# Godotcoffee/AlignGraph2

Hardware: AMD Instinct MI355X
Metric: aligned-read-bases/sec through PAGraph build+traverse (higher is better)
Workload: dtype u32

## Files before the change

aligngraph2_amd/capi.py:

```python
import ctypes as C

import numpy as np

CONSTANTS = {
    "PAG_OK": 0, "PAG_EINVAL": -22, "PAG_ENOMEM": -12, "PAG_ENODEV": -19, "PAG_ERANGE": -34, "PAG_EFAULT": -14, "PAG_EDOM": -33,
    "PAG_NONE": 0xFFFFFFFF,
    "PAG_ALN_REV_STRAND": 1, "PAG_ALN_WALK_BACK": 2, "PAG_ALN_ELIGIBLE": 4,
    "PAG_ORIENT_NONE": -1, "PAG_ORIENT_REVERSE": 0, "PAG_ORIENT_FORWARD": 1, "PAG_ORIENT_BOTH": 2,
    "PAG_TRAVEL_RENDER_DUMPS": 1, "PAG_TRAVEL_RENDER_SEQS": 2,
}
globals().update(CONSTANTS)

DTYPES = {
    "pag_aln": np.dtype([("query", "<u4"), ("target", "<u4"), ("t_begin", "<u4"), ("t_end", "<u4"), ("q_start", "<u4"),
                         ("t_start", "<u4"), ("n_cols", "<u4"), ("n_valid", "<u4"), ("diff_off", "<u8"), ("flags", "<u4"),
                         ("reserved", "<u4")]),
    "pag_ctg": np.dtype([("len", "<u4"), ("selected", "<u4"), ("single_base", "<u4"), ("multi", "<u4"), ("map_off", "<u8")]),
    "pag_ref": np.dtype([("len", "<u4"), ("accepted", "<u4"), ("single_base", "<u4"), ("reserved", "<u4")]),
    "pag_raw_aln": np.dtype([("query", "<u4"), ("target", "<u4"), ("score", "<u8"), ("q_begin", "<u8"), ("q_end", "<u8"),
                             ("t_begin", "<u8"), ("t_end", "<u8"), ("diff_off", "<u8"), ("n_cols", "<u4"), ("n_emit", "<u4"),
                             ("n_radv", "<u4"), ("forward", "<u4")]),
    "pag_path_node": np.dtype([("code", "<u4"), ("ctg", "<u4"), ("ref", "<u4"), ("cnt", "<u2"), ("reserved", "<u2"),
                               ("step", "<i4"), ("vid", "<u4")]),
}

_u32, _i32, _u64, _f64, _vp = C.c_uint32, C.c_int32, C.c_uint64, C.c_double, C.c_void_p


class PagSeqs(C.Structure):
    _c_name_ = "pag_seqs"
    _fields_ = [("n_seqs", _u64), ("byte_off", _vp), ("len", _vp), ("packed", _vp), ("packed_bytes", _u64)]


class PagAlnDb(C.Structure):
    _c_name_ = "pag_aln_db"
    _fields_ = [("n_aln", _u64), ("aln", _vp), ("query_off", _vp), ("diff", _vp), ("n_diff_words", _u64)]


class PagBuildInput(C.Structure):
    _c_name_ = "pag_build_input"
    _fields_ = [("on_device", _u32), ("n_threads", _u32), ("reads", PagSeqs), ("emit_order", _vp), ("read_to_ctg", PagAlnDb),
                ("read_to_ref", PagAlnDb), ("n_ctgs", _u64), ("ctgs", _vp), ("ctg_ent_off", _vp), ("n_ctg_ent_off", _u64),
                ("ctg_ent", _vp), ("n_ctg_ent", _u64), ("n_refs", _u64), ("refs", _vp), ("eps", _u32), ("cov_filter", _u32),
                ("outer_sample", _u32), ("topk_ctg", _i32), ("topk_ref", _i32), ("reserved", _u32)]


class PagRawDb(C.Structure):
    _c_name_ = "pag_raw_db"
    _fields_ = [("n", _u64), ("rec", _vp), ("diff", _vp), ("n_diff_words", _u64)]


class PagRawInput(C.Structure):
    _c_name_ = "pag_raw_input"
    _fields_ = [("bulk_on_device", _u32), ("n_threads", _u32), ("reads", PagSeqs), ("read_to_ctg", PagRawDb),
                ("read_to_ref", PagRawDb), ("ctg_to_ref", PagRawDb), ("n_ctgs", _u64), ("ctg_len", _vp), ("ctg_selected", _vp),
                ("ctg_forward", _vp), ("n_refs", _u64), ("ref_len", _vp), ("ref_accepted", _vp), ("read_to_ctg_ratio", _f64),
                ("read_to_ref_ratio", _f64), ("eps", _u32), ("cov_filter", _u32), ("outer_sample", _u32), ("topk_ctg", _i32),
                ("topk_ref", _i32), ("reserved", _u32)]


class BuildStats(C.Structure):
    _c_name_ = "pag_build_stats"
    _fields_ = [("merge_edge", _u64 * 2), ("total_pos", _u64 * 2), ("merge_pos", _u64 * 2), ("n_tuples", _u64 * 2),
                ("n_edges", _u64 * 2), ("n_nodes", _u64), ("n_pos", _u64), ("n_uniq_edges", _u64), ("ms_extract", _f64),
                ("ms_sort", _f64), ("ms_cluster", _f64), ("ms_edges", _f64), ("ms_total", _f64), ("ms_sort_kernel", _f64),
                ("sort_records", _u64)]

    def counts(self):
        return (self.merge_edge[0], self.total_pos[0], self.merge_pos[0], self.merge_edge[1], self.total_pos[1],
                self.merge_pos[1])


class Csr(C.Structure):
    _c_name_ = "pag_csr"
    _fields_ = [("n_nodes", _u64), ("n_pos", _u64), ("n_edges", _u64), ("node_code", _vp), ("pos_off", _vp), ("pos_ctg", _vp),
                ("pos_ref", _vp), ("pos_cnt", _vp), ("edge_off", _vp), ("edge_to", _vp), ("edge_step", _vp)]


class ShardSlice(C.Structure):
    _c_name_ = "pag_shard_slice"
    _fields_ = [("n_t", _u64), ("n_e", _u64), ("tkey", _vp), ("tval", _vp), ("tseg", _vp), ("tcnt", _vp), ("ekey", _vp),
                ("eval", _vp), ("eseg", _vp), ("stats", BuildStats)]


class Region(C.Structure):
    _c_name_ = "pag_region"
    _fields_ = [("n_ctg_iv", _u64), ("ctg_iv", _vp), ("n_ref_iv", _u64), ("ref_iv", _vp), ("ref_open", _vp)]


class TravelParams(C.Structure):
    _c_name_ = "pag_travel_params"
    _fields_ = [("ref_threads", _u32), ("reserved", _u32), ("deviation", _u64), ("error_rate", _f64), ("start_split", _f64),
                ("min_len", _u64)]


class TravelStats(C.Structure):
    _c_name_ = "pag_travel_stats"
    _fields_ = [("ms_compact", _f64), ("ms_walk", _f64), ("ms_total", _f64), ("rounds", _u64), ("jobs", _u64),
                ("walk_steps", _u64), ("classify_calls", _u64), ("probes", _u64), ("records", _u64)]


class PagSucc(C.Structure):
    _c_name_ = "pag_succ"
    _fields_ = [("code", _u32), ("step", _u32), ("pos", _u64), ("grade", _u32), ("ctg_similar", _u32)]


class CnsAln(C.Structure):
    _c_name_ = "pag_cns_aln"
    _fields_ = [("str_off", _u64), ("len", _u32), ("start", _u32), ("weight", _i32), ("reserved", _u32)]


class CnsPart(C.Structure):
    _c_name_ = "pag_cns_part"
    _fields_ = [("bb_off", _u64), ("bb_len", _u32), ("n_aln", _u32), ("aln_first", _u64), ("node_cap", _u32),
                ("edge_cap", _u32), ("aux_cap", _u32), ("out_cap", _u32)]


class KmerCountResult(C.Structure):
    _c_name_ = "pag_kmer_count_result"
    _fields_ = [("min_abundance", _u64), ("n_solid", _u64), ("n_kmers_counted", _u64), ("ms_count", _f64), ("ms_select", _f64)]


class TraverseStats(C.Structure):
    _c_name_ = "pagh_traverse_stats"
    _fields_ = [("n_contigs", _u64), ("n_path_nodes", _u64), ("n_path_bases", _u64), ("n_chains_emitted", _u64),
                ("n_fasta_bases", _u64), ("path_checksum", _u64), ("ms_export", _f64), ("ms_traverse", _f64), ("ms_total", _f64),
                ("ms_successors", _f64), ("ms_walk", _f64), ("walk_rounds", _u64), ("walk_jobs", _u64), ("walk_steps", _u64),
                ("walk_classifications", _u64)]


STRUCTS = {s._c_name_: s for s in (PagSeqs, PagAlnDb, PagBuildInput, PagRawDb, PagRawInput, BuildStats, Csr, ShardSlice, Region,
                                   TravelParams, TravelStats, PagSucc, CnsAln, CnsPart, KmerCountResult, TraverseStats)}

NOT_MIRRORED = {}

_int, _i64, _cs = C.c_int, C.c_int64, C.c_char_p
_u64p, _i64p, _intp = C.POINTER(_u64), C.POINTER(_i64), C.POINTER(_int)
_stats, _slice, _region = C.POINTER(BuildStats), C.POINTER(ShardSlice), C.POINTER(Region)
_traverse = [_vp, _u32, _vp, _vp, _vp, _vp, _vp, _u32, _u64, _u64, _cs, _cs, _u32, _vp]
_cns = [_int, _cs, _u64, _vp, _u64, _vp, _u64, _cs, _cs, _u64, _i32, _vp, _u64, _vp, _vp, _vp]

SIGNATURES = {
    "pag_create": (_vp, [_vp, _u64, _u32, _int, _intp]),
    "pag_create_from_bitmap": (_vp, [_vp, _u64, _u32, _int, _int, _intp]),
    "pag_destroy": (None, [_vp]),
    "pag_solid_count": (_u64, [_vp]),
    "pag_reset": (_int, [_vp]),
    "pag_process": (_int, [_vp, _vp, _vp]),
    "pag_prepare": (_int, [_vp, _vp, _vp]),
    "pag_shard_extract": (_int, [_vp, _vp, _u32, _u32, _u64p]),
    "pag_shard_extract_range": (_int, [_vp, _vp, _u64, _u64, _u32, _u64p]),
    "pag_shard_take": (_int, [_vp, _vp, _vp, _vp, _vp]),
    "pag_shard_take_part": (_int, [_vp, _u64, _u64, _vp, _vp, _u64, _u64, _vp, _vp]),
    "pag_shard_build": (_int, [_vp, _vp, _vp, _u64, _u64, _vp, _vp, _u64, _u64, _u32, _stats]),
    "pag_shard_export": (_int, [_vp, _slice]),
    "pag_shard_take_slice": (_int, [_vp, _vp, _vp, _vp, _vp, _vp, _vp, _vp]),
    "pag_shard_import": (_int, [_vp, _slice, _u32, _stats]),
    "pag_shard_select": (_int, [_vp, _region, _slice]),
    "pag_shard_set_region": (_int, [_vp, _region]),
    "pag_shard_release_build": (_int, [_vp]),
    "pag_shard_adopt": (_int, [_vp, _u64, _u64, _stats]),
    "pag_comm_create": (_vp, [_int, _int, _cs, _int, _cs, _intp]),
    "pag_comm_destroy": (None, [_vp]),
    "pag_comm_rank": (_int, [_vp]),
    "pag_comm_world": (_int, [_vp]),
    "pag_comm_bytes_sent": (_u64, [_vp]),
    "pag_comm_abort": (None, [_vp, _cs]),
    "pag_comm_barrier": (_int, [_vp]),
    "pag_comm_all_gather": (_int, [_vp, _vp, _u64, _vp]),
    "pag_comm_gather_v": (_int, [_vp, _vp, _u64, _int, _vp, _u64, _vp, _vp]),
    "pag_comm_all_to_all_v": (_int, [_vp, _vp, _vp, _vp, _vp]),
    "pag_shard_run": (_int, [_vp, _vp, _vp, _vp, _stats]),
    "pag_csr_sizes": (_int, [_vp, _u64p, _u64p, _u64p]),
    "pag_export_csr": (_int, [_vp, _vp]),
    "pag_travel_prepare": (_int, [_vp, _vp, _vp, _u64, _vp, _vp]),
    "pag_travel_prepare_for": (_int, [_vp, _vp, _vp, _vp, _u64, _vp, _vp]),
    "pag_travel_view_sizes": (_int, [_vp, _vp, _vp, _vp, _vp, _vp, _vp]),
    "pag_travel": (_int, [_vp, _vp, _vp, _vp, _u64, _vp, _vp]),
    "pag_successors": (_i64, [_vp, _u32, _u64, _vp, _u64]),
    "pag_travel_path": (_vp, [_vp, _u64, _u64p]),
    "pag_travel_path_oriented": (_vp, [_vp, _u64, _int, _u64p]),
    "pag_reserve_walk_arena": (_int, [_vp, _u64]),
    "pag_render_dump_lines": (_int, [_vp, _u64, _u32, _vp, _u64, _vp, _u64, _vp, _u64, _u64p, _int]),
    "pag_travel_dump_text": (_vp, [_vp, _u64, _int, _u64p]),
    "pag_render_path_sequence": (_int, [_vp, _u64, _u32, _vp, _vp, _u64, _f64, _vp, _u64, _u64p, _int]),
    "pag_travel_seq_sources": (_int, [_vp, _vp]),
    "pag_travel_seq_text": (_vp, [_vp, _u64, _int, _u64p]),
    "pag_pack_text_seqs": (_int, [_vp, _int, _u64, _vp, _vp, _u64, _vp, _vp, _u64, _int]),
    "pag_classify_columns": (_int, [_vp, _int, _u64, _vp, _vp, _vp, _vp, _vp, _u64, _vp, _u64, _vp, _vp, _int]),
    "pag_classify_columns_host": (_int, [_vp, _u64, _vp, _vp, _vp, _vp, _vp, _u64, _vp, _u64, _vp, _vp, _int]),
    "pag_cns_consensus": (_int, _cns),
    "pag_cns_consensus_wave": (_int, _cns),
    "pag_kmer_count": (_int, [_vp, _int, _u32, _f64, _int, _vp, _int, _vp]),
    "pag_last_error": (_cs, []),
    "pag_device_available": (_int, []),
    "pag_device_warm": (_int, [_int]),
    "pagh_traverse": (_int, _traverse),
    "pagh_traverse_begin": (_int, [_vp, _u32, _vp, _vp, _vp, _vp, _vp, _u32, _u64, _u64, _cs, _cs, _u32]),
    "pagh_traverse_end": (_int, [_vp, _vp]),
    "pagh_assemble_paths": (_int, [_vp, _u32, _vp, _vp, _vp, _vp, _vp, _vp, _vp, _u32, _u64, _u64, _cs, _cs, _u32, _vp]),
    "pagh_assemble_paths_text": (_int, [_vp, _u32, _vp, _vp, _vp, _vp, _vp, _vp, _vp, _vp, _vp, _u32, _u64, _u64, _cs, _cs, _u32,
                                        _vp]),
    "pagh_assemble_paths_seq": (_int, [_vp, _u32, _vp, _vp, _vp, _vp, _vp, _vp, _vp, _vp, _vp, _vp, _vp, _u32, _u64, _u64, _cs, _cs,
                                       _u32, _vp]),
    "pagh_release": (None, [_vp]),
    "pagh_last_error": (_cs, []),
    "pag_debug_edit_distance": (_u64, [_cs, _cs]),
    "pag_debug_mapper_d2s": (_u64, [_vp, _u64, _i64, _i64]),
    "pag_debug_mapper_s2d": (None, [_vp, _u64, _u64, _i64p, _i64p]),
    "pag_debug_mapper_extra": (_u64, [_vp, _u64]),
    "pag_debug_succ_sizes": (_int, [_vp, _vp, _vp]),
    "pag_debug_succ": (_int, [_vp, _vp, _vp]),
    "pag_debug_trav_vertices": (_int, [_vp, _vp, _vp]),
    "pag_debug_stream_sizes": (_int, [_vp, _u64p, _u64p]),
    "pag_debug_streams": (_int, [_vp, _vp, _vp, _vp, _vp]),
    "pag_debug_cov_filter": (_int, [_vp, _u64, _vp, _u64, _u32, _vp, _int]),
    "pag_debug_predicates": (_int, [_vp, _u64, _f64, _vp, _vp, _int]),
    "pag_debug_predicates_tab": (_int, [_vp, _u64, _f64, _vp, _vp, _int, _vp]),
    "pagh_debug_classify_columns": (None, [_cs, _u64, _cs, _u64, _vp, _vp, _vp, _int]),
    "pagh_debug_pack_bases": (None, [_cs, _u64, _vp, _int]),
}


def bind(lib, rename=None):
    for name, (restype, argtypes) in SIGNATURES.items():
        sym = rename(name) if rename else name
        fn = getattr(lib, sym, None) if sym else None
        if fn is not None:
            fn.restype = restype
            fn.argtypes = list(argtypes)
    return lib
```

aligngraph2_amd/csrc/hip/k5_travel_host.hip:

```cpp
#include <algorithm>
#include <atomic>
#include <chrono>
#include <cmath>
#include <cstdio>
#include <cstdlib>
#include <cstring>
#include <deque>
#include <string>
#include <thread>
#include <unordered_set>
#include <vector>

#include "pag_graph_impl.hpp"
#include "pagraph_debug.h"
#include "walk_config.hpp"
#include "walk_stitch.hpp"
#include "walker_grid.hpp"

using namespace pagdev;

namespace {

#include "trav_prepare_host.hpp"
#include "walk_session_jobs.hpp"
#include "walk_session_rounds.hpp"
#include "walk_session_loop.hpp"


}


extern "C" {

uint64_t pag_debug_edit_distance(const char *a, const char *b) { return edit_distance(a, b); }
uint64_t pag_debug_mapper_d2s(const uint32_t *len, uint64_t n, int64_t idx, int64_t pos) { return Mapper(len, n).dualToSingle(idx, pos); }
void pag_debug_mapper_s2d(const uint32_t *len, uint64_t n, uint64_t single, int64_t *idx, int64_t *pos) {
    auto d = Mapper(len, n).singleToDual(single);
    *idx = d.first;
    *pos = d.second;
}
uint64_t pag_debug_mapper_extra(const uint32_t *len, uint64_t n) { return Mapper(len, n).starts.back(); }

const pag_path_node *pag_travel_path_oriented(const pag_graph *g, uint64_t ctg_index, int forward, uint64_t *len) {
    const uint64_t slot = 2 * ctg_index + (forward ? 0 : 1);
    if (!g || slot >= g->path_valid.size() || !g->path_valid[slot]) {
        if (len) *len = 0;
        return nullptr;
    }
    if (len) *len = g->path_len[slot];
    if (slot < g->path_ptr.size() && g->path_ptr[slot]) return g->path_ptr[slot];
    return g->path_store + g->path_off[slot];
}

const char *pag_travel_dump_text(const pag_graph *g, uint64_t ctg_index, int forward, uint64_t *bytes) {
    const uint64_t slot = 2 * ctg_index + (forward ? 0 : 1);
    if (bytes) *bytes = 0;
    if (!g || slot >= g->path_valid.size() || !g->path_valid[slot] || slot >= g->text_ptr.size() || !g->text_ptr[slot]) return nullptr;
    if (bytes) *bytes = g->text_len[slot];
    return g->text_ptr[slot];
}

const char *pag_travel_seq_text(const pag_graph *g, uint64_t ctg_index, int forward, uint64_t *bytes) {
    const uint64_t slot = 2 * ctg_index + (forward ? 0 : 1);
    if (bytes) *bytes = 0;
    if (!g || slot >= g->path_valid.size() || !g->path_valid[slot] || slot >= g->seq_ptr.size() || !g->seq_ptr[slot]) return nullptr;
    if (bytes) *bytes = g->seq_len[slot];
    return g->seq_ptr[slot];
}
int pag_travel_seq_sources(pag_graph *g, const pag_seqs *refs) {
    if (!g) return PAG_EINVAL;
    g->seq_refs = refs;
    return PAG_OK;
}

const pag_path_node *pag_travel_path(const pag_graph *g, uint64_t ctg_index, uint64_t *len) {
    if (g && 2 * ctg_index + 1 < g->path_valid.size() && !g->path_valid[2 * ctg_index]) return pag_travel_path_oriented(g, ctg_index, 0, len);
    return pag_travel_path_oriented(g, ctg_index, 1, len);
}

int pag_debug_succ_sizes(const pag_graph *g, uint64_t *n_pos, uint64_t *n_succ) {
    if (!g || !g->tg_ready || !n_pos || !n_succ) return PAG_EINVAL;
    *n_pos = g->tg.n_pos;
    *n_succ = g->tg.n_succ;
    return PAG_OK;
}
int pag_debug_succ(const pag_graph *g, uint32_t *succ_off, void *recs) {
    if (!g || !g->tg_ready || !succ_off || !recs) return PAG_EINVAL;
    PAG_HIP_TRY(hipSetDevice(g->device));
    PAG_HIP_TRY(hipMemcpy(succ_off, g->tg.succ_off, (g->tg.n_pos + 1) * 4, hipMemcpyDeviceToHost));
    PAG_HIP_TRY(hipMemcpy(recs, g->tg.succ, g->tg.n_succ * sizeof(SuccRec), hipMemcpyDeviceToHost));
    return PAG_OK;
}

int pag_debug_trav_vertices(const pag_graph *g, uint32_t *code, uint64_t *pos) {
    if (!g || !g->tg_ready || !code || !pos) return PAG_EINVAL;
    PAG_HIP_TRY(hipSetDevice(g->device));
    const TravGraph &G = g->tg;
    std::vector<uint32_t> uold(G.n_pos), vnode(G.n_pos), ncode(G.n_nodes);
    PAG_HIP_TRY(hipMemcpy(uold.data(), G.uold, G.n_pos * 4, hipMemcpyDeviceToHost));
    PAG_HIP_TRY(hipMemcpy(vnode.data(), G.vnode, G.n_pos * 4, hipMemcpyDeviceToHost));
    PAG_HIP_TRY(hipMemcpy(ncode.data(), G.ncode, G.n_nodes * 4, hipMemcpyDeviceToHost));
    PAG_HIP_TRY(hipMemcpy(pos, G.upos, G.n_pos * 8, hipMemcpyDeviceToHost));
    for (uint64_t u = 0; u < G.n_pos; ++u) code[u] = ncode[vnode[uold[u]]];
    return PAG_OK;
}

int64_t pag_successors(const pag_graph *g, uint32_t code, uint64_t pos, pag_succ *out, uint64_t cap) {
    if (!g || !g->tg_ready || (!out && cap)) return PAG_EINVAL;
    PAG_HIP_TRY(hipSetDevice(g->device));
    if (g->view_pruned || g->regional) {
        set_error("pag_successors: the prepared view was cut for given traversals (pag_travel_prepare_for / a regional graph): its lists are restricted to what those traversals can examine");
        return PAG_ERANGE;
    }
    void *d = nullptr;
    const uint64_t room = std::min<uint64_t>(cap, g->tg.n_succ);
    PAG_HIP_TRY(hipMalloc(&d, 16 + room * sizeof(pag_succ)));
    unsigned long long *d_n = (unsigned long long *)d;
    void *d_recs = (char *)d + 16;
    int rc = trav_successors_of(g->tg, code, pos, d_recs, room, d_n, g->stream);
    unsigned long long n = 0;
    if (rc == PAG_OK && (hipMemcpyAsync(&n, d_n, 8, hipMemcpyDeviceToHost, g->stream) != hipSuccess || hipStreamSynchronize(g->stream) != hipSuccess)) rc = PAG_EFAULT;
    if (rc == PAG_OK && n == ~0ull) {
        set_error("pag_successors: the graph holds no vertex with that k-mer and position");
        rc = PAG_EINVAL;
    } else if (rc == PAG_OK && n == ~1ull) {
        set_error("pag_successors: that vertex's list is a marker record");
        rc = PAG_ERANGE;
    } else if (rc == PAG_OK && std::min<uint64_t>(n, room) &&
               hipMemcpy(out, d_recs, std::min<uint64_t>(n, room) * sizeof(pag_succ), hipMemcpyDeviceToHost) != hipSuccess) {
        rc = PAG_EFAULT;
    }
    hipFree(d);
    return rc == PAG_OK ? (int64_t)n : rc;
}

int pag_travel_prepare(pag_graph *g, const pag_seqs *ctgs, const uint32_t *ref_len, uint64_t n_refs, const pag_travel_params *prm, double *ms) {
    return pag_travel_prepare_for(g, ctgs, nullptr, ref_len, n_refs, prm, ms);
}
int pag_travel_prepare_for(pag_graph *g, const pag_seqs *ctgs, const int32_t *orient, const uint32_t *ref_len, uint64_t n_refs,
                           const pag_travel_params *prm, double *ms) {
    if (!g || !ctgs || !prm || (!ref_len && n_refs)) return PAG_EINVAL;
    PAG_HIP_TRY(hipSetDevice(g->device));
    TravGraph G{};
    return trav_prepare_graph(g, ctgs->len, ctgs->n_seqs, ref_len, n_refs, prm->deviation, prm->error_rate, &G, ms, orient, prm->start_split);
}
int pag_travel_view_sizes(const pag_graph *g, uint64_t *n_nodes, uint64_t *n_pos, uint64_t *n_edges, uint64_t *n_succ, int *cut, uint64_t *fallbacks) {
    if (!g || !g->tg_ready) return PAG_EINVAL;
    if (n_nodes) *n_nodes = g->view_counts[0];
    if (n_pos) *n_pos = g->view_counts[1];
    if (n_edges) *n_edges = g->view_counts[2];
    if (n_succ) *n_succ = g->tg.n_succ;
    if (cut) *cut = g->view_pruned ? 1 : 0;
    if (fallbacks) *fallbacks = g->view_fallbacks;
    return PAG_OK;
}

static int travel_once(pag_graph *g, const pag_seqs *ctgs, const int32_t *orient, const uint32_t *ref_len, uint64_t n_refs,
                       const pag_travel_params *prm, pag_travel_stats *stats);
int pag_travel(pag_graph *g, const pag_seqs *ctgs, const int32_t *orient, const uint32_t *ref_len, uint64_t n_refs,
               const pag_travel_params *prm, pag_travel_stats *stats) {
    if (!g || !ctgs || !orient || !prm || (!ref_len && n_refs)) return PAG_EINVAL;
    int rc = travel_once(g, ctgs, orient, ref_len, n_refs, prm, stats);
    if (rc == PAG_ERANGE && g->view_pruned && !g->regional) {
        if (WalkConfig::from_env().timing) std::fprintf(stderr, "[timing] a walk left the view: %s; walking again on the whole graph\n", pag_last_error());
        g->view_off = true;
        g->tg_ready = false;
        g->view_fallbacks += 1;
        rc = travel_once(g, ctgs, orient, ref_len, n_refs, prm, stats);
    }
    g->seq_refs = nullptr;
    return rc;
}
static int travel_once(pag_graph *g, const pag_seqs *ctgs, const int32_t *orient, const uint32_t *ref_len, uint64_t n_refs,
                       const pag_travel_params *prm, pag_travel_stats *stats) {
    WalkSession W(g, ctgs, orient, ref_len, n_refs, prm, stats);
    return W.run();
}


}
```

aligngraph2_amd/csrc/hip/k5_view.hip:

```cpp
#include <algorithm>
#include <cmath>
#include <cstring>
#include <string>
#include <vector>

#include "pag_device.hpp"
#include "pag_travel.hpp"
#include "trav_device.hpp"

namespace pagdev {

__device__ __forceinline__ bool iv_contains(const uint32_t *__restrict__ iv, uint32_t n, uint32_t x, uint32_t *which = nullptr) {
    if (!n) return false;
    uint32_t lo = 0, hi = n;
    while (hi - lo > 1) {
        const uint32_t mid = (lo + hi) >> 1;
        if (iv[2 * mid] <= x) lo = mid;
        else hi = mid;
    }
    if (which) *which = lo;
    return x >= iv[2 * lo] && x < iv[2 * lo + 1];
}
constexpr uint32_t ZONE_LDS = 2048;
__global__ void k_zone_bands(const uint64_t *__restrict__ tval, uint64_t T, const uint32_t *__restrict__ zones, uint32_t n_z,
                             uint32_t *__restrict__ lo, uint32_t *__restrict__ hi) {
    __shared__ uint32_t s_lo[ZONE_LDS], s_hi[ZONE_LDS], s_z[2 * ZONE_LDS];
    const bool lds = n_z <= ZONE_LDS;
    if (lds) {
        for (uint32_t z = threadIdx.x; z < n_z; z += blockDim.x) {
            s_lo[z] = 0xFFFFFFFFu;
            s_hi[z] = 0u;
            s_z[2 * z] = zones[2 * z];
            s_z[2 * z + 1] = zones[2 * z + 1];
        }
        __syncthreads();
    }
    const uint32_t z_first = n_z ? zones[0] : 0u, z_last = n_z ? zones[2 * n_z - 1] : 0u;
    for (uint64_t i = (uint64_t)blockIdx.x * blockDim.x + threadIdx.x; i < T; i += (uint64_t)gridDim.x * blockDim.x) {
        const uint64_t p = tval[i];
        const uint32_t c = (uint32_t)(p >> 32), r = (uint32_t)p;
        uint32_t z;
        if (c < z_first || c >= z_last || r == 0u) continue;
        if (!(lds ? iv_contains(s_z, n_z, c, &z) : iv_contains(zones, n_z, c, &z))) continue;
        if (lds) {
            atomicMin(&s_lo[z], r);
            atomicMax(&s_hi[z], r);
        } else {
            atomicMin(&lo[z], r);
            atomicMax(&hi[z], r);
        }
    }
    if (lds) {
        __syncthreads();
        for (uint32_t z = threadIdx.x; z < n_z; z += blockDim.x)
            if (s_hi[z] != 0u) {
                atomicMin(&lo[z], s_lo[z]);
                atomicMax(&hi[z], s_hi[z]);
            }
    }
}
constexpr uint32_t PRUNE_LDS = 4096;
constexpr uint32_t VC_T = 256, VC_R = 8, VC_TILE = VC_T * VC_R, VC_W = VC_T / 64;
__global__ __launch_bounds__(VC_T) void k_view_mark(const uint32_t *__restrict__ tkey, const uint64_t *__restrict__ tval, const uint32_t *__restrict__ tseg,
                                                    uint64_t T, const uint32_t *__restrict__ civ, uint32_t n_civ, const uint32_t *__restrict__ riv,
                                                    uint32_t n_riv, int whole, uint64_t *__restrict__ ballots, uint32_t *__restrict__ tile_first,
                                                    uint32_t *__restrict__ tile_keep, uint64_t n_tiles) {
    __shared__ uint32_t s_iv[PRUNE_LDS];
    __shared__ uint32_t s_ck[VC_R][VC_W], s_pk[VC_R][VC_W], s_cf[VC_R][VC_W];
    __shared__ uint16_t s_pre[VC_TILE];
    const bool lds = !whole && 2u * (n_civ + n_riv) <= PRUNE_LDS;
    if (lds) {
        for (uint32_t x = threadIdx.x; x < 2u * n_civ; x += blockDim.x) s_iv[x] = civ[x];
        for (uint32_t x = threadIdx.x; x < 2u * n_riv; x += blockDim.x) s_iv[2u * n_civ + x] = riv[x];
        __syncthreads();
    }
    auto inside = [&](uint64_t p) {
        const uint32_t c = (uint32_t)(p >> 32), r = (uint32_t)p;
        if (whole) return true;
        if (lds) return c != 0u ? iv_contains(s_iv, n_civ, c) : iv_contains(s_iv + 2u * n_civ, n_riv, r);
        return c != 0u ? iv_contains(civ, n_civ, c) : iv_contains(riv, n_riv, r);
    };
    const uint32_t lane = lane_id(), w = threadIdx.x >> 6;
    for (uint64_t tile = blockIdx.x; tile < n_tiles; tile += gridDim.x) {
        const uint64_t tile_base = tile * VC_TILE;
        uint32_t kb = 0;
        uint32_t off_r[VC_R];
        uint64_t bkr[VC_R];
#pragma unroll
        for (uint32_t r = 0; r < VC_R; ++r) {
            const uint64_t i = tile_base + (uint64_t)r * VC_T + threadIdx.x;
            bool kk = false;
            off_r[r] = 0;
            if (i < T) {
                const uint32_t kx = tkey[i], v = tseg[i];
                const bool head = i == 0 || tkey[i - 1] != kx;
                const bool leader = head ? v != 0u : (v & SEG_LEADER) != 0u;
                if (leader) {
                    kk = inside(tval[i]);
                    off_r[r] = head ? 0u : (v & ~SEG_LEADER);
                }
            }
            bkr[r] = __ballot(kk);
            kb |= kk ? 1u << r : 0u;
            if (lane == 0) s_ck[r][w] = (uint32_t)__popcll(bkr[r]);
        }
        __syncthreads();
        if (threadIdx.x == 0) {
            uint32_t ak = 0;
            for (uint32_t r = 0; r < VC_R; ++r)
                for (uint32_t ww = 0; ww < VC_W; ++ww) {
                    s_pk[r][ww] = ak;
                    ak += s_ck[r][ww];
                }
            tile_keep[tile] = ak;
        }
        __syncthreads();
#pragma unroll
        for (uint32_t r = 0; r < VC_R; ++r)
            s_pre[r * VC_T + threadIdx.x] = (uint16_t)(s_pk[r][w] + (uint32_t)__popcll(bkr[r] & lanemask_lt()));
        __syncthreads();
#pragma unroll
        for (uint32_t r = 0; r < VC_R; ++r) {
            const uint32_t d = r * VC_T + threadIdx.x;
            bool ff = false;
            if ((kb >> r) & 1u) {
                const uint32_t off = off_r[r];
                if (off <= d) {
                    ff = s_pre[d] == s_pre[d - off];
                } else {
                    ff = s_pre[d] == 0u;
                    const uint64_t i = tile_base + d;
                    for (uint64_t j = i - off; j < tile_base && ff; ++j) {
                        const uint32_t kx = tkey[j], v = tseg[j];
                        const bool head = j == 0 || tkey[j - 1] != kx;
                        const bool leader = head ? v != 0u : (v & SEG_LEADER) != 0u;
                        ff = !(leader && inside(tval[j]));
                    }
                }
            }
            const uint64_t bf = __ballot(ff);
            if (lane == 0) {
                s_cf[r][w] = (uint32_t)__popcll(bf);
                const uint64_t at = ((tile * VC_R + r) * VC_W + w) * 2u;
                ballots[at] = bkr[r];
                ballots[at + 1] = bf;
            }
        }
        __syncthreads();
        if (threadIdx.x == 0) {
            uint32_t af = 0;
            for (uint32_t r = 0; r < VC_R; ++r)
                for (uint32_t ww = 0; ww < VC_W; ++ww) af += s_cf[r][ww];
            tile_first[tile] = af;
        }
    }
}
__global__ __launch_bounds__(VC_T) void k_view_write(const uint32_t *__restrict__ tkey, const uint64_t *__restrict__ tval, const uint16_t *__restrict__ tcnt,
                                                     const uint64_t *__restrict__ ballots, const uint64_t *__restrict__ base_first,
                                                     const uint64_t *__restrict__ base_keep, uint64_t n_tiles, TravGraph G) {
    __shared__ uint64_t s_b[VC_R * VC_W * 2];
    __shared__ uint32_t s_pk[VC_R][VC_W], s_pf[VC_R][VC_W];
    const uint32_t w = threadIdx.x >> 6;
    for (uint64_t tile = blockIdx.x; tile < n_tiles; tile += gridDim.x) {
        if (threadIdx.x < VC_R * VC_W * 2) s_b[threadIdx.x] = ballots[tile * (VC_R * VC_W * 2) + threadIdx.x];
        __syncthreads();
        if (threadIdx.x == 0) {
            uint32_t ak = 0, af = 0;
            for (uint32_t r = 0; r < VC_R; ++r)
                for (uint32_t ww = 0; ww < VC_W; ++ww) {
                    s_pk[r][ww] = ak;
                    s_pf[r][ww] = af;
                    ak += (uint32_t)__popcll(s_b[(r * VC_W + ww) * 2]);
                    af += (uint32_t)__popcll(s_b[(r * VC_W + ww) * 2 + 1]);
                }
        }
        __syncthreads();
        const uint64_t bk0 = base_keep[tile], bf0 = base_first[tile];
#pragma unroll
        for (uint32_t r = 0; r < VC_R; ++r) {
            const uint64_t bk = s_b[(r * VC_W + w) * 2], bf = s_b[(r * VC_W + w) * 2 + 1];
            const uint64_t me = 1ull << lane_id();
            if (!(bk & me)) continue;
            const bool ff = (bf & me) != 0ull;
            const uint64_t i = tile * VC_TILE + (uint64_t)r * VC_T + threadIdx.x;
            const uint64_t p = bk0 + s_pk[r][w] + (uint32_t)__popcll(bk & lanemask_lt());
            const uint64_t n = bf0 + s_pf[r][w] + (uint32_t)__popcll(bf & lanemask_lt()) + (ff ? 1u : 0u) - 1u;
            G.vpos[p] = tval[i];
            G.vcnt[p] = tcnt[i];
            G.vnode[p] = (uint32_t)n;
            if (ff) {
                const uint32_t kx = tkey[i];
                G.ncode[n] = kx;
                G.npos_off[n] = (uint32_t)p;
                atomicOr((unsigned long long *)&G.bitmap[kx >> 6], 1ull << (kx & 63u));
            }
        }
        __syncthreads();
    }
}

__global__ void k_popc_words(const uint64_t *__restrict__ bitmap, uint64_t n_words, uint32_t *__restrict__ out) {
    for (uint64_t i = (uint64_t)blockIdx.x * blockDim.x + threadIdx.x; i < n_words; i += (uint64_t)gridDim.x * blockDim.x)
        out[i] = (uint32_t)__popcll(bitmap[i]);
}

__global__ void k_narrow(const uint64_t *__restrict__ in, uint64_t n, uint32_t *__restrict__ out) {
    for (uint64_t i = (uint64_t)blockIdx.x * blockDim.x + threadIdx.x; i < n; i += (uint64_t)gridDim.x * blockDim.x)
        out[i] = (uint32_t)in[i];
}

__global__ void k_edge_counts(const uint32_t *__restrict__ ekey, const uint32_t *__restrict__ eseg, uint64_t E, TravGraph G,
                              uint32_t *__restrict__ necnt) {
    for (uint64_t j = (uint64_t)blockIdx.x * blockDim.x + threadIdx.x; j < E; j += (uint64_t)gridDim.x * blockDim.x) {
        uint32_t kx = ekey[j];
        if (j != 0 && ekey[j - 1] == kx) continue;
        uint32_t n = node_of_code(G, kx);
        if (n != PAG_NONE) necnt[n] = eseg[j];
    }
}

__global__ void k_code_table(TravGraph G, uint64_t *__restrict__ tab) {
    for (uint64_t n = (uint64_t)blockIdx.x * blockDim.x + threadIdx.x; n < G.n_nodes; n += (uint64_t)gridDim.x * blockDim.x) {
        const U32x2 r = *(const U32x2 *)(G.npos_off + n);
        tab[G.ncode[n]] = (uint64_t)r.a[0] | ((uint64_t)(r.a[1] - r.a[0]) << 32);
    }
}

__global__ void k_compact_edges(const uint32_t *__restrict__ ekey, const uint64_t *__restrict__ eval,
                                const uint32_t *__restrict__ eseg, uint64_t E, TravGraph G, const uint64_t *__restrict__ tab) {
    for (uint64_t j = (uint64_t)blockIdx.x * blockDim.x + threadIdx.x; j < E; j += (uint64_t)gridDim.x * blockDim.x) {
        uint32_t kx = ekey[j];
        if (j != 0 && ekey[j - 1] == kx) continue;
        uint32_t n = node_of_code(G, kx);
        if (n == PAG_NONE) continue;
        uint32_t dst = G.nedge_off[n], len = eseg[j];
        for (uint32_t l0 = 0; l0 < len; l0 += 4u) {
            uint64_t v4[4];
            uint32_t p04[4], q4[4];
#pragma unroll
            for (uint32_t t = 0; t < 4u; ++t) v4[t] = l0 + t < len ? eval[j + l0 + t] : 0ull;
            if (tab) {
                uint64_t e4[4];
#pragma unroll
                for (uint32_t t = 0; t < 4u; ++t) e4[t] = l0 + t < len ? tab[(uint32_t)(v4[t] >> 32)] : ~0ull;
#pragma unroll
                for (uint32_t t = 0; t < 4u; ++t) {
                    p04[t] = (uint32_t)e4[t];
                    q4[t] = (uint32_t)(e4[t] >> 32);
                }
            } else {
                uint32_t to4[4];
                U32x2 r4[4];
#pragma unroll
                for (uint32_t t = 0; t < 4u; ++t) to4[t] = l0 + t < len ? node_of_code(G, (uint32_t)(v4[t] >> 32)) : PAG_NONE;
#pragma unroll
                for (uint32_t t = 0; t < 4u; ++t) r4[t] = *(const U32x2 *)(G.npos_off + (to4[t] != PAG_NONE ? to4[t] : 0u));
#pragma unroll
                for (uint32_t t = 0; t < 4u; ++t) {
                    p04[t] = to4[t] != PAG_NONE ? r4[t].a[0] : PAG_NONE;
                    q4[t] = r4[t].a[1] - r4[t].a[0];
                }
            }
#pragma unroll
            for (uint32_t t = 0; t < 4u; ++t) {
                const uint32_t l = l0 + t;
                if (l >= len) break;
                const uint32_t step = (((uint32_t)v4[t]) >> 1) & EDGE_STEP_MASK;
                if (p04[t] == PAG_NONE) {
                    G.eto[dst + l] = PAG_NONE;
                    G.estep[dst + l] = step;
                } else {
                    G.eto[dst + l] = p04[t];
                    G.estep[dst + l] = step | ((q4[t] < EDGE_Q_MANY ? q4[t] : EDGE_Q_MANY) << 24);
                }
            }
        }
    }
}

__global__ void k_ctg_nodes(const uint8_t *__restrict__ packed, const TravCtgNodesJob *__restrict__ jobs, uint32_t k, TravGraph G,
                            uint32_t *__restrict__ out_all) {
    const TravCtgNodesJob J = jobs[blockIdx.y];
    const uint32_t len = J.len;
    const bool forward = J.forward != 0;
    uint32_t *__restrict__ out = out_all + J.out_off;
    const uint32_t n_pos = len >= k ? len - k + 1 : 0;
    const uint32_t kmask = k >= 16 ? 0xFFFFFFFFu : ((1u << (2 * k)) - 1u);
    const uint32_t *words = (const uint32_t *)(packed + J.byte_off);
    for (uint32_t i = blockIdx.x * blockDim.x + threadIdx.x; i < n_pos; i += gridDim.x * blockDim.x) {
        uint32_t a = forward ? i : len - k - i;
        uint32_t w = a >> 4, sh = (a & 15u) * 2u;
        uint64_t W = (uint64_t)words[w] | ((uint64_t)words[w + 1] << 32);
        uint32_t x = (uint32_t)(W >> sh) & kmask;
        uint32_t code = forward ? (rev2(x) >> (32 - 2 * k)) : ((~x) & kmask);
        out[i] = node_of_code(G, code);
    }
}

__global__ void k_order_keys(const uint64_t *__restrict__ vpos, uint64_t n, uint32_t *__restrict__ key, uint64_t *__restrict__ val) {
    for (uint64_t i = (uint64_t)blockIdx.x * blockDim.x + threadIdx.x; i < n; i += (uint64_t)gridDim.x * blockDim.x) {
        const uint64_t p = vpos[i];
        key[i] = (uint32_t)(p >> 32);
        val[i] = (p << 32) | i;
    }
}

__global__ void k_order_apply(const uint32_t *__restrict__ sorted_ctg, const uint64_t *__restrict__ sorted_val, uint64_t n, uint64_t n_zero, TravGraph G,
                              uint32_t slice, uint32_t slice_shift) {
    for (uint64_t u = (uint64_t)blockIdx.x * blockDim.x + threadIdx.x; u < n; u += (uint64_t)gridDim.x * blockDim.x) {
        uint32_t v;
        if (slice == 0u) {
            const uint64_t x = sorted_val[u];
            v = (uint32_t)x;
            G.uold[u] = v;
            G.upos[u] = ((uint64_t)(u < n_zero ? 0u : sorted_ctg[u]) << 32) | (x >> 32);
        } else {
            v = G.uold[u];
        }
        if (slice_shift >= 32u || (v >> slice_shift) == slice) {
            G.newid[v] = (uint32_t)u;
            G.ucnt[u] = G.vcnt[v];
        }
    }
}

int trav_compact(const uint32_t *tkey, const uint64_t *tval, const uint32_t *tseg, const uint16_t *tcnt, uint64_t T,
                 const uint32_t *ekey, const uint64_t *eval, const uint32_t *eseg, uint64_t E, uint32_t k, uint64_t n_nodes,
                 uint64_t n_pos, uint64_t n_edges, TravGraph G, void *tmp, size_t tmp_bytes, hipStream_t s, const TravView *view,
                 uint64_t *counts_out) {
    const uint64_t n_words = ((1ull << (2 * k)) + 63) / 64;
    const uint64_t n_tiles_all = (T + VC_TILE - 1) / VC_TILE;
    const uint64_t m = std::max(n_tiles_all, std::max(n_words, n_nodes + 1)) + 1;
    const uint64_t m_ballots = n_tiles_all * (VC_TILE / 64 * 2 + 1) + 64;
    char *p = (char *)tmp;
    auto take = [&](size_t bytes) {
        char *q = p;
        p += (bytes + 255) & ~(size_t)255;
        return (void *)q;
    };
    uint32_t *flags = (uint32_t *)take(m * 4);
    uint64_t *sc1 = (uint64_t *)take(m * 8);
    uint64_t *sc2 = (uint64_t *)take(m_ballots * 8);
    uint32_t *keep = (uint32_t *)take((n_tiles_all + 1) * 4);
    uint64_t *totals = (uint64_t *)take(64);
    void *scan_tmp = take(scan_tmp_bytes(m));
    uint64_t *code_tab = k <= TRAV_CODE_TABLE_MAX_K ? (uint64_t *)take((size_t)8 << (2 * k)) : nullptr;
    if ((size_t)(p - (char *)tmp) > tmp_bytes) {
        set_error("trav_compact: scratch too small");
        return PAG_EINVAL;
    }
    PAG_HIP_TRY(hipMemsetAsync(G.bitmap, 0, n_words * 8, s));
    int rc;
    if (T) {
        const uint64_t n_tiles = (T + VC_TILE - 1) / VC_TILE;
        uint32_t *tile_first = flags, *tile_keep = keep;
        const unsigned grid = (unsigned)std::min<uint64_t>(n_tiles, 256u * 8u);
        const uint32_t *civ = view ? view->civ : nullptr, *riv = view ? view->riv : nullptr;
        const uint32_t n_civ = view ? view->n_civ : 0u, n_riv = view ? view->n_riv : 0u;
        uint64_t *ballots = sc2 + n_tiles + 16;
        k_view_mark<<<dim3(grid), dim3(VC_T), 0, s>>>(tkey, tval, tseg, T, civ, n_civ, riv, n_riv, view ? 0 : 1, ballots, tile_first, tile_keep, n_tiles);
        if ((rc = scan_u32_to_u64(tile_first, sc1, n_tiles, totals, scan_tmp, s))) return rc;
        if ((rc = scan_u32_to_u64(tile_keep, sc2, n_tiles, totals + 1, scan_tmp, s))) return rc;
        k_view_write<<<dim3(grid), dim3(VC_T), 0, s>>>(tkey, tval, tcnt, ballots, sc1, sc2, n_tiles, G);
    }
    if (view) {
        uint64_t h[2] = {0, 0};
        if (T) {
            PAG_HIP_TRY(hipMemcpyAsync(h, totals, 16, hipMemcpyDeviceToHost, s));
            PAG_HIP_TRY(hipStreamSynchronize(s));
        }
        if (h[0] > n_nodes || h[1] > n_pos) {
            set_error("trav_compact: the view holds more than the graph");
            return PAG_EFAULT;
        }
        n_nodes = h[0];
        n_pos = h[1];
        G.n_nodes = n_nodes;
        G.n_pos = n_pos;
    }
    uint32_t np32 = (uint32_t)n_pos;
    PAG_HIP_TRY(hipMemcpyAsync(G.npos_off + n_nodes, &np32, 4, hipMemcpyHostToDevice, s));
    k_popc_words<<<dim3(grid_for(n_words)), dim3(256), 0, s>>>(G.bitmap, n_words, flags);
    if ((rc = scan_u32_to_u64(flags, sc1, n_words, nullptr, scan_tmp, s))) return rc;
    k_narrow<<<dim3(grid_for(n_words)), dim3(256), 0, s>>>(sc1, n_words, G.rank);
    PAG_HIP_TRY(hipMemsetAsync(flags, 0, (n_nodes + 1) * 4, s));
    if (E) k_edge_counts<<<dim3(grid_for(E)), dim3(256), 0, s>>>(ekey, eseg, E, G, flags);
    if ((rc = scan_u32_to_u64(flags, sc1, n_nodes + 1, view ? totals + 2 : nullptr, scan_tmp, s))) return rc;
    k_narrow<<<dim3(grid_for(n_nodes + 1)), dim3(256), 0, s>>>(sc1, n_nodes + 1, G.nedge_off);
    if (E && code_tab) {
        PAG_HIP_TRY(hipMemsetAsync(code_tab, 0xFF, (size_t)8 << (2 * k), s));
        TravGraph Gn = G;
        Gn.n_nodes = n_nodes;
        if (n_nodes) k_code_table<<<dim3(grid_for(n_nodes)), dim3(256), 0, s>>>(Gn, code_tab);
    }
    if (E) k_compact_edges<<<dim3(grid_for(E)), dim3(256), 0, s>>>(ekey, eval, eseg, E, G, code_tab);
    if (view) {
        uint64_t ne = 0;
        PAG_HIP_TRY(hipMemcpyAsync(&ne, totals + 2, 8, hipMemcpyDeviceToHost, s));
        PAG_HIP_TRY(hipStreamSynchronize(s));
        if (ne > n_edges) {
            set_error("trav_compact: the view holds more edges than the graph");
            return PAG_EFAULT;
        }
        n_edges = ne;
    }
    if (counts_out) {
        counts_out[0] = n_nodes;
        counts_out[1] = n_pos;
        counts_out[2] = n_edges;
    }
    PAG_HIP_TRY(hipGetLastError());
    return PAG_OK;
}

size_t trav_compact_tmp_bytes(uint64_t T, uint64_t E, uint32_t k, uint64_t n_nodes) {
    (void)E;
    const uint64_t n_words = ((1ull << (2 * k)) + 63) / 64;
    const uint64_t n_tiles = (T + VC_TILE - 1) / VC_TILE;
    const uint64_t m = std::max(n_tiles, std::max(n_words, n_nodes + 1)) + 1, m_ballots = n_tiles * (VC_TILE / 64 * 2 + 1) + 64;
    auto al = [](size_t b) { return (b + 255) & ~(size_t)255; };
    return al(m * 4) + al(m * 8) + al(m_ballots * 8) + al((n_tiles + 1) * 4) + al(64) + al(scan_tmp_bytes(m)) + (k <= TRAV_CODE_TABLE_MAX_K ? al((size_t)8 << (2 * k)) : 0) + 1024;
}

int trav_zone_bands(const uint64_t *tval, uint64_t T, const uint32_t *zones_dev, uint32_t n_z, uint32_t *lo_dev, uint32_t *hi_dev, hipStream_t s) {
    if (!n_z) return PAG_OK;
    PAG_HIP_TRY(hipMemsetAsync(lo_dev, 0xFF, (size_t)n_z * 4, s));
    PAG_HIP_TRY(hipMemsetAsync(hi_dev, 0, (size_t)n_z * 4, s));
    if (T) k_zone_bands<<<dim3(grid_for(T)), dim3(256), 0, s>>>(tval, T, zones_dev, n_z, lo_dev, hi_dev);
    PAG_HIP_TRY(hipGetLastError());
    return PAG_OK;
}

void trav_launch_ctg_nodes(const uint8_t *packed, const TravCtgNodesJob *jobs, uint32_t n_jobs, uint32_t max_len, uint32_t k, TravGraph G, uint32_t *out,
                           hipStream_t s) {
    const uint32_t n = max_len >= k ? max_len - k + 1 : 0;
    if (!n || !n_jobs) return;
    for (uint32_t at = 0; at < n_jobs; at += 65535u) {
        const uint32_t m = std::min(n_jobs - at, 65535u);
        k_ctg_nodes<<<dim3(std::min(grid_for(n), 256u), m), dim3(256), 0, s>>>(packed, jobs + at, k, G, out);
    }
}

__global__ void k_max_step(const uint32_t *__restrict__ estep, uint64_t n, uint32_t *__restrict__ out) {
    uint32_t m = 0;
    for (uint64_t i = (uint64_t)blockIdx.x * blockDim.x + threadIdx.x; i < n; i += (uint64_t)gridDim.x * blockDim.x) m = (estep[i] & EDGE_STEP_MASK) > m ? (estep[i] & EDGE_STEP_MASK) : m;
    m = wave_max_u32(m);
    if (lane_id() == 0 && m) atomicMax(out, m);
}
__global__ void k_mark_incomplete(TravGraph G, uint32_t n_zero, const uint32_t *__restrict__ iv, const uint8_t *__restrict__ open, uint32_t n_iv,
                                  uint32_t margin, uint32_t *__restrict__ bits) {
    const uint64_t u = (uint64_t)blockIdx.x * blockDim.x + threadIdx.x;
    bool bad = false;
    if (u < G.n_pos) bad = d_incomplete_by_position(iv, open, n_iv, margin, (uint32_t)G.upos[u], u >= n_zero);
    const uint64_t m = __ballot(bad);
    if ((threadIdx.x & 63u) == 0 && u < ((G.n_pos + 63ull) & ~63ull)) {
        bits[u >> 5] = (uint32_t)m;
        bits[(u >> 5) + 1] = (uint32_t)(m >> 32);
    }
}
int trav_mark_incomplete(TravGraph &G, uint32_t n_zero, const uint32_t *iv_host, const uint8_t *open_host, uint32_t n_iv, uint32_t dev, double err,
                         uint32_t *bits, void *tmp, hipStream_t s) {
    uint32_t *d_max = (uint32_t *)tmp;
    uint32_t *d_iv = d_max + 64;
    uint8_t *d_open = (uint8_t *)(d_iv + 2 * (size_t)n_iv + 2);
    PAG_HIP_TRY(hipMemsetAsync(d_max, 0, 4, s));
    if (G.n_edges) k_max_step<<<dim3(grid_for(G.n_edges)), dim3(256), 0, s>>>(G.estep, G.n_edges, d_max);
    if (n_iv) {
        PAG_HIP_TRY(hipMemcpyAsync(d_iv, iv_host, 2 * (size_t)n_iv * 4, hipMemcpyHostToDevice, s));
        PAG_HIP_TRY(hipMemcpyAsync(d_open, open_host, 2 * (size_t)n_iv, hipMemcpyHostToDevice, s));
    }
    uint32_t max_step = 0;
    PAG_HIP_TRY(hipMemcpyAsync(&max_step, d_max, 4, hipMemcpyDeviceToHost, s));
    PAG_HIP_TRY(hipStreamSynchronize(s));
    const uint64_t margin = (uint64_t)((double)max_step * (1.0 + err)) + dev + 2;
    const bool bits_read = n_iv > INC_LDS_MAX;
    if (G.n_pos && bits_read) k_mark_incomplete<<<dim3((unsigned)((G.n_pos + 255) / 256)), dim3(256), 0, s>>>(G, n_zero, d_iv, d_open, n_iv, (uint32_t)std::min<uint64_t>(margin, 0x7FFFFFFFu), bits);
    PAG_HIP_TRY(hipGetLastError());
    G.incomplete = bits;
    G.inc_iv = d_iv;
    G.inc_open = d_open;
    G.inc_n = n_iv;
    G.inc_margin = (uint32_t)std::min<uint64_t>(margin, 0x7FFFFFFFu);
    return PAG_OK;
}
size_t trav_mark_incomplete_tmp_bytes(uint32_t n_iv) { return 256 + (2 * (size_t)n_iv + 2) * 4 + 2 * (size_t)n_iv + 64; }

__global__ void k_zero_prefix(const uint32_t *__restrict__ key, uint64_t n, unsigned long long *__restrict__ n0) {
    for (uint64_t i = (uint64_t)blockIdx.x * blockDim.x + threadIdx.x; i < n; i += (uint64_t)gridDim.x * blockDim.x)
        if (key[i] == 0u && (i + 1 == n || key[i + 1] != 0u)) *n0 = i + 1;
}
__global__ void k_order_refkeys(const uint64_t *__restrict__ val, uint64_t n, uint32_t *__restrict__ key) {
    for (uint64_t i = (uint64_t)blockIdx.x * blockDim.x + threadIdx.x; i < n; i += (uint64_t)gridDim.x * blockDim.x)
        key[i] = (uint32_t)(val[i] >> 32);
}

int trav_order(TravGraph G, uint32_t *key, uint64_t *val, uint32_t *key2, uint64_t *val2, void *sort_tmp, uint64_t *n_zero, int ctg_bits,
               int ref_bits, hipStream_t s) {
    const uint64_t n = G.n_pos;
    if (n_zero) *n_zero = 0;
    if (!n) return PAG_OK;
    k_order_keys<<<dim3(grid_for(n)), dim3(256), 0, s>>>(G.vpos, n, key, val);
    int in0 = 1, rc;
    if ((rc = sort_pairs(key, val, key2, val2, n, ctg_bits, sort_tmp, &in0, s, nullptr, nullptr))) return rc;
    uint32_t *ks = in0 ? key : key2, *ko = in0 ? key2 : key;
    uint64_t *vs = in0 ? val : val2, *vo = in0 ? val2 : val;
    unsigned long long *d_n0 = (unsigned long long *)sort_tmp;
    unsigned long long n0 = 0;
    PAG_HIP_TRY(hipMemsetAsync(d_n0, 0, 8, s));
    k_zero_prefix<<<dim3(grid_for(n)), dim3(256), 0, s>>>(ks, n, d_n0);
    PAG_HIP_TRY(hipMemcpyAsync(&n0, d_n0, 8, hipMemcpyDeviceToHost, s));
    PAG_HIP_TRY(hipStreamSynchronize(s));
    if (n0 > 1) {
        k_order_refkeys<<<dim3(grid_for(n0)), dim3(256), 0, s>>>(vs, n0, ks);
        int in0b = 1;
        if ((rc = sort_pairs(ks, vs, ko, vo, n0, ref_bits, sort_tmp, &in0b, s, nullptr, nullptr))) return rc;
        if (!in0b) PAG_HIP_TRY(hipMemcpyAsync(vs, vo, n0 * 8, hipMemcpyDeviceToDevice, s));
    }
    if (n_zero) *n_zero = n0;
    {
        uint32_t lg = n >= (32ull << 20) ? 3u : 0u;
        if (const long long want = env_int("PAG_ORDER_SLICES", 0)) {
            lg = 0;
            while ((1u << (lg + 1)) <= (uint32_t)std::max<long long>(1, want)) ++lg;
        }
        uint32_t bits = 1;
        while (bits < 32 && (n >> bits) != 0) ++bits;
        if (lg >= bits) lg = 0;
        const uint32_t shift = lg ? bits - lg : 32u;
        for (uint32_t sl = 0; sl < (1u << lg); ++sl)
            k_order_apply<<<dim3(grid_for(n)), dim3(256), 0, s>>>(ks, vs, n, n0 > 1 ? n0 : 0, G, sl, shift);
    }
    PAG_HIP_TRY(hipGetLastError());
    return PAG_OK;
}

}
```

include/pagraph_debug.h:

```cpp
#ifndef PAGRAPH_DEBUG_H
#define PAGRAPH_DEBUG_H

#include "pagraph_hip.h"

#ifdef __cplusplus
extern "C" {
#endif

uint64_t pag_debug_edit_distance(const char *a, const char *b);
uint64_t pag_debug_mapper_d2s(const uint32_t *len, uint64_t n, int64_t idx, int64_t pos);
void pag_debug_mapper_s2d(const uint32_t *len, uint64_t n, uint64_t single, int64_t *idx, int64_t *pos);
uint64_t pag_debug_mapper_extra(const uint32_t *len, uint64_t n);
int pag_debug_succ_sizes(const pag_graph *g, uint64_t *n_pos, uint64_t *n_succ);
int pag_debug_succ(const pag_graph *g, uint32_t *succ_off, void *recs);
int pag_debug_trav_vertices(const pag_graph *g, uint32_t *code, uint64_t *pos);
int pag_debug_stream_sizes(const pag_graph *g, uint64_t *n_tuples, uint64_t *n_edges);
int pag_debug_streams(const pag_graph *g, uint32_t *tkey, uint64_t *tval, uint32_t *ekey, uint64_t *eval);
int pag_debug_cov_filter(const pag_aln *aln, uint64_t n_aln, const pag_ref *refs, uint64_t n_refs, uint32_t cov_filter,
                         uint8_t *ok, int device);
int pag_debug_predicates(const uint32_t *rows, uint64_t n, double err, uint8_t *grade, uint8_t *edge_sim, int device);
int pag_debug_predicates_tab(const uint32_t *rows, uint64_t n, double err, uint8_t *grade, uint8_t *edge_sim, int device,
                             uint64_t *n_through_table);

void pagh_debug_classify_columns(const char *q, uint64_t n, const char *r, uint64_t rn, uint32_t *words, uint32_t *n_emit,
                                 uint32_t *n_radv, int scalar_only);
void pagh_debug_pack_bases(const char *sq, uint64_t n, uint8_t *out, int scalar_only);

#ifdef __cplusplus
}
#endif
#endif
```

Baseline: 4.197 billion.

## Merge two-pass vertex ordering sort into one composite-key radix sort

Vertex ordering previously sorted by contig id, counted the zero-contig prefix with a host sync, and then re-sorted that prefix by reference position. The keys now carry a flag bit: zero-contig vertices keep their ref position and the rest get flag|contig. A single radix sort over B+1 bits then does the job when that fits in the same number of byte passes, and the zero count comes from a ballot in the key kernel. This removes the second sort, the prefix kernel and a mid-pipeline host sync, at the cost of possibly more radix passes for the main sort and an n_zero counter stored just past the val buffer. Debug accessors for traversal edges are also added.

```diff
diff --git a/aligngraph2_amd/capi.py b/aligngraph2_amd/capi.py
--- a/aligngraph2_amd/capi.py
+++ b/aligngraph2_amd/capi.py
@@ -212,6 +212,8 @@
     "pag_debug_succ_sizes": (_int, [_vp, _vp, _vp]),
     "pag_debug_succ": (_int, [_vp, _vp, _vp]),
     "pag_debug_trav_vertices": (_int, [_vp, _vp, _vp]),
+    "pag_debug_trav_edges_sizes": (_int, [_vp, _vp, _vp]),
+    "pag_debug_trav_edges": (_int, [_vp, _vp, _vp, _vp]),
     "pag_debug_stream_sizes": (_int, [_vp, _u64p, _u64p]),
     "pag_debug_streams": (_int, [_vp, _vp, _vp, _vp, _vp]),
     "pag_debug_cov_filter": (_int, [_vp, _u64, _vp, _u64, _u32, _vp, _int]),
diff --git a/aligngraph2_amd/csrc/hip/k5_travel_host.hip b/aligngraph2_amd/csrc/hip/k5_travel_host.hip
--- a/aligngraph2_amd/csrc/hip/k5_travel_host.hip
+++ b/aligngraph2_amd/csrc/hip/k5_travel_host.hip
@@ -105,6 +105,22 @@
     return PAG_OK;
 }
 
+int pag_debug_trav_edges_sizes(const pag_graph *g, uint64_t *n_nodes, uint64_t *n_edges) {
+    if (!g || !g->tg_ready || !n_nodes || !n_edges) return PAG_EINVAL;
+    *n_nodes = g->tg.n_nodes;
+    *n_edges = g->tg.n_edges;
+    return PAG_OK;
+}
+int pag_debug_trav_edges(const pag_graph *g, uint32_t *nedge_off, uint32_t *eto, uint32_t *estep) {
+    if (!g || !g->tg_ready || !nedge_off || !eto || !estep) return PAG_EINVAL;
+    PAG_HIP_TRY(hipSetDevice(g->device));
+    const TravGraph &G = g->tg;
+    PAG_HIP_TRY(hipMemcpy(nedge_off, G.nedge_off, (G.n_nodes + 1) * 4, hipMemcpyDeviceToHost));
+    PAG_HIP_TRY(hipMemcpy(eto, G.eto, G.n_edges * 4, hipMemcpyDeviceToHost));
+    PAG_HIP_TRY(hipMemcpy(estep, G.estep, G.n_edges * 4, hipMemcpyDeviceToHost));
+    return PAG_OK;
+}
+
 int64_t pag_successors(const pag_graph *g, uint32_t code, uint64_t pos, pag_succ *out, uint64_t cap) {
     if (!g || !g->tg_ready || (!out && cap)) return PAG_EINVAL;
     PAG_HIP_TRY(hipSetDevice(g->device));
diff --git a/aligngraph2_amd/csrc/hip/k5_view.hip b/aligngraph2_amd/csrc/hip/k5_view.hip
--- a/aligngraph2_amd/csrc/hip/k5_view.hip
+++ b/aligngraph2_amd/csrc/hip/k5_view.hip
@@ -297,23 +297,40 @@
     }
 }
 
-__global__ void k_order_keys(const uint64_t *__restrict__ vpos, uint64_t n, uint32_t *__restrict__ key, uint64_t *__restrict__ val) {
-    for (uint64_t i = (uint64_t)blockIdx.x * blockDim.x + threadIdx.x; i < n; i += (uint64_t)gridDim.x * blockDim.x) {
-        const uint64_t p = vpos[i];
-        key[i] = (uint32_t)(p >> 32);
-        val[i] = (p << 32) | i;
-    }
-}
-
-__global__ void k_order_apply(const uint32_t *__restrict__ sorted_ctg, const uint64_t *__restrict__ sorted_val, uint64_t n, uint64_t n_zero, TravGraph G,
-                              uint32_t slice, uint32_t slice_shift) {
+__global__ void k_order_keys(const uint64_t *__restrict__ vpos, uint64_t n, uint32_t flag, uint32_t *__restrict__ key, uint64_t *__restrict__ val,
+                             unsigned long long *__restrict__ n_zero) {
+    const uint64_t n_up = (n + 63ull) & ~63ull;
+    unsigned long long zeros = 0;
+    for (uint64_t i = (uint64_t)blockIdx.x * blockDim.x + threadIdx.x; i < n_up; i += (uint64_t)gridDim.x * blockDim.x) {
+        bool zero = false;
+        if (i < n) {
+            const uint64_t p = vpos[i];
+            const uint32_t c = (uint32_t)(p >> 32);
+            zero = c == 0u;
+            key[i] = flag == 0u ? c : zero ? (uint32_t)p : flag | c;
+            val[i] = (p << 32) | i;
+        }
+        if (flag != 0u) zeros += (unsigned long long)__popcll(__ballot(zero));
+    }
+    if (flag != 0u && lane_id() == 0 && zeros) atomicAdd(n_zero, zeros);
+}
+
+__global__ void k_order_apply(const uint32_t *__restrict__ sorted_ctg, const uint64_t *__restrict__ sorted_val, uint64_t n, uint64_t n_zero, uint32_t flag,
+                              TravGraph G, uint32_t slice, uint32_t slice_shift) {
     for (uint64_t u = (uint64_t)blockIdx.x * blockDim.x + threadIdx.x; u < n; u += (uint64_t)gridDim.x * blockDim.x) {
         uint32_t v;
         if (slice == 0u) {
             const uint64_t x = sorted_val[u];
             v = (uint32_t)x;
             G.uold[u] = v;
-            G.upos[u] = ((uint64_t)(u < n_zero ? 0u : sorted_ctg[u]) << 32) | (x >> 32);
+            uint32_t c;
+            if (flag != 0u) {
+                const uint32_t kx = sorted_ctg[u];
+                c = (kx & flag) ? kx & (flag - 1u) : 0u;
+            } else {
+                c = u < n_zero ? 0u : sorted_ctg[u];
+            }
+            G.upos[u] = ((uint64_t)c << 32) | (x >> 32);
         } else {
             v = G.uold[u];
         }
@@ -499,24 +516,37 @@
     const uint64_t n = G.n_pos;
     if (n_zero) *n_zero = 0;
     if (!n) return PAG_OK;
-    k_order_keys<<<dim3(grid_for(n)), dim3(256), 0, s>>>(G.vpos, n, key, val);
+    const int B = std::max(ctg_bits, ref_bits);
+    bool one_sort = B < 32 && (B + 1 + 7) / 8 <= (ctg_bits + 7) / 8;
+    if (const long long want = env_int("PAG_ORDER_SORTS", 0)) {
+        if (want == 1 && B >= 32) {
+            set_error("trav_order: PAG_ORDER_SORTS=1, but 32-bit coordinates leave no room for the flag bit of the composite key");
+            return PAG_EINVAL;
+        }
+        one_sort = want == 1;
+    }
+    const uint32_t flag = one_sort ? 1u << B : 0u;
+    unsigned long long *d_n0 = one_sort ? (unsigned long long *)(val + n) : (unsigned long long *)sort_tmp;
+    unsigned long long n0 = 0;
+    if (one_sort) PAG_HIP_TRY(hipMemsetAsync(d_n0, 0, 8, s));
+    k_order_keys<<<dim3(grid_for(n)), dim3(256), 0, s>>>(G.vpos, n, flag, key, val, d_n0);
     int in0 = 1, rc;
-    if ((rc = sort_pairs(key, val, key2, val2, n, ctg_bits, sort_tmp, &in0, s, nullptr, nullptr))) return rc;
+    if ((rc = sort_pairs(key, val, key2, val2, n, one_sort ? B + 1 : ctg_bits, sort_tmp, &in0, s, nullptr, nullptr))) return rc;
     uint32_t *ks = in0 ? key : key2, *ko = in0 ? key2 : key;
     uint64_t *vs = in0 ? val : val2, *vo = in0 ? val2 : val;
-    unsigned long long *d_n0 = (unsigned long long *)sort_tmp;
-    unsigned long long n0 = 0;
-    PAG_HIP_TRY(hipMemsetAsync(d_n0, 0, 8, s));
-    k_zero_prefix<<<dim3(grid_for(n)), dim3(256), 0, s>>>(ks, n, d_n0);
-    PAG_HIP_TRY(hipMemcpyAsync(&n0, d_n0, 8, hipMemcpyDeviceToHost, s));
-    PAG_HIP_TRY(hipStreamSynchronize(s));
-    if (n0 > 1) {
-        k_order_refkeys<<<dim3(grid_for(n0)), dim3(256), 0, s>>>(vs, n0, ks);
-        int in0b = 1;
-        if ((rc = sort_pairs(ks, vs, ko, vo, n0, ref_bits, sort_tmp, &in0b, s, nullptr, nullptr))) return rc;
-        if (!in0b) PAG_HIP_TRY(hipMemcpyAsync(vs, vo, n0 * 8, hipMemcpyDeviceToDevice, s));
-    }
-    if (n_zero) *n_zero = n0;
+    if (!one_sort) {
+        PAG_HIP_TRY(hipMemsetAsync(d_n0, 0, 8, s));
+        k_zero_prefix<<<dim3(grid_for(n)), dim3(256), 0, s>>>(ks, n, d_n0);
+        PAG_HIP_TRY(hipMemcpyAsync(&n0, d_n0, 8, hipMemcpyDeviceToHost, s));
+        PAG_HIP_TRY(hipStreamSynchronize(s));
+        if (n0 > 1) {
+            k_order_refkeys<<<dim3(grid_for(n0)), dim3(256), 0, s>>>(vs, n0, ks);
+            int in0b = 1;
+            if ((rc = sort_pairs(ks, vs, ko, vo, n0, ref_bits, sort_tmp, &in0b, s, nullptr, nullptr))) return rc;
+            if (!in0b) PAG_HIP_TRY(hipMemcpyAsync(vs, vo, n0 * 8, hipMemcpyDeviceToDevice, s));
+        }
+        if (n_zero) *n_zero = n0;
+    }
     {
         uint32_t lg = n >= (32ull << 20) ? 3u : 0u;
         if (const long long want = env_int("PAG_ORDER_SLICES", 0)) {
@@ -528,9 +558,14 @@
         if (lg >= bits) lg = 0;
         const uint32_t shift = lg ? bits - lg : 32u;
         for (uint32_t sl = 0; sl < (1u << lg); ++sl)
-            k_order_apply<<<dim3(grid_for(n)), dim3(256), 0, s>>>(ks, vs, n, n0 > 1 ? n0 : 0, G, sl, shift);
+            k_order_apply<<<dim3(grid_for(n)), dim3(256), 0, s>>>(ks, vs, n, n0 > 1 ? n0 : 0, flag, G, sl, shift);
     }
     PAG_HIP_TRY(hipGetLastError());
+    if (one_sort) {
+        PAG_HIP_TRY(hipMemcpyAsync(&n0, d_n0, 8, hipMemcpyDeviceToHost, s));
+        PAG_HIP_TRY(hipStreamSynchronize(s));
+        if (n_zero) *n_zero = n0;
+    }
     return PAG_OK;
 }
 
diff --git a/include/pagraph_debug.h b/include/pagraph_debug.h
--- a/include/pagraph_debug.h
+++ b/include/pagraph_debug.h
@@ -14,6 +14,8 @@
 int pag_debug_succ_sizes(const pag_graph *g, uint64_t *n_pos, uint64_t *n_succ);
 int pag_debug_succ(const pag_graph *g, uint32_t *succ_off, void *recs);
 int pag_debug_trav_vertices(const pag_graph *g, uint32_t *code, uint64_t *pos);
+int pag_debug_trav_edges_sizes(const pag_graph *g, uint64_t *n_nodes, uint64_t *n_edges);
+int pag_debug_trav_edges(const pag_graph *g, uint32_t *nedge_off, uint32_t *eto, uint32_t *estep);
 int pag_debug_stream_sizes(const pag_graph *g, uint64_t *n_tuples, uint64_t *n_edges);
 int pag_debug_streams(const pag_graph *g, uint32_t *tkey, uint64_t *tval, uint32_t *ekey, uint64_t *eval);
 int pag_debug_cov_filter(const pag_aln *aln, uint64_t n_aln, const pag_ref *refs, uint64_t n_refs, uint32_t cov_filter,
```

Result: slower. 4.076 billion (-2.9%).
